# DanielQ-51/cudapathtracer

Hardware: AMD Instinct MI355X
Metric: Mray/s (higher is better)
Workload: dtype f32; 1 GPU; cornell_1920x1080_1024spp_depth8_mis; spp=1024, max_depth=8, integrator=UNIDIRECTIONAL (MIS), variant=megakernel, seed=103033, triangles=36, bvh_nodes=31

## Files before the change

cudapathtracer_amd/api.py:

```python
from __future__ import annotations

import ctypes as C
import os

import numpy as np

_HERE = os.path.dirname(os.path.abspath(__file__))
LIB_PATH = os.environ.get("PT_LIB_PATH") or os.path.join(_HERE, "csrc", "libptamd.so")

UNIDIRECTIONAL = 0
NAIVE_UNIDIRECTIONAL = 2
SEED = 103033
INFO_KEYS = ("width", "height", "spp", "max_depth", "integrator", "leaf_size", "n_tris", "n_lights", "n_nodes",
             "n_points", "n_normals", "n_uvs", "n_mats", "largest_leaf", "backup_count", "tree_depth")
COUNTER_KEYS = ("rays_closest", "rays_shadow", "node_pops", "box_tests", "tri_tests", "hits", "rng_draws", "iterations")


class _F4(C.Union):
    _fields_ = [("v", C.c_float * 4), ("_align", C.c_longdouble)]


class Camera(C.Structure):

    _fields_ = [("cameraOrigin", _F4), ("w", C.c_int32), ("h", C.c_int32), ("xRot", C.c_float), ("yRot", C.c_float),
# ... 140 lines not shown
    L.pt_preview_motion.argtypes = [vp]
    L.pt_preview_set_motion_chain.argtypes = [vp, i32]
    L.pt_preview_motion_chain.argtypes = [vp]
    L.pt_render_ids.argtypes = [vp, C.POINTER(Camera), i32, i32, i32, vp]
    L.pt_render_ids_device.argtypes = [vp, C.POINTER(Camera), i32, i32, i32, vp, vp]
    L.pt_pick.argtypes = [vp, C.POINTER(Camera), i32, i32, i32, vp, i32, vp, vp]
    L.pt_select_overlay.argtypes = [i32, i32, vp, i32, C.POINTER(SelectEntry), vp]
    L.pt_select_overlay_device.argtypes = [i32, i32, vp, i32, C.POINTER(SelectEntry), vp, vp]
    L.pt_preview_set_selection.argtypes = [vp, i32, C.POINTER(SelectEntry), i32]
    L.pt_preview_pick.argtypes = [vp, i32, i32, i32, vp, vp]
    L.pt_preview_read_ids.argtypes = [vp, vp]
    L.pt_preview_device_ids.restype = vp; L.pt_preview_device_ids.argtypes = [vp]
    L.pt_preview_id_passes.argtypes = [vp]
    L.pt_debug_update_ms.argtypes = [vp, vp]
    L.pt_light_triangles.argtypes = [C.POINTER(SceneDesc), vp]
    L.pt_scene_destroy.argtypes = [vp]
    L.pt_render.argtypes = [vp, C.POINTER(Camera), i32, i32, i32, i32, i32, i32, u64, C.POINTER(TileRange), vp]
    L.pt_render_counted.argtypes = [vp, C.POINTER(Camera), i32, i32, i32, i32, i32, i32, u64, C.POINTER(TileRange), vp, vp]
    L.pt_render_tiles_device.argtypes = [vp, C.POINTER(Camera), i32, i32, i32, i32, i32, i32, u64, C.POINTER(TileRange), vp, i32, vp]
    L.pt_untile_device.argtypes = [i32, i32, C.POINTER(TileRange), vp, vp, vp]
    L.pt_tile_device.argtypes = [i32, i32, C.POINTER(TileRange), vp, vp, vp]
    L.pt_launch_unidirectional.argtypes = [i32, Camera, vp, i32, i32, i32, i32, vp]
    L.pt_launch_naive_unidirectional.argtypes = [i32, Camera, vp, i32, i32, i32, i32, vp]
    L.pt_set_variant.argtypes = [vp, i32]
    L.pt_has_experimental.restype = i32
    L.pt_get_counters.argtypes = [vp, vp]
    L.pt_reset_counters.argtypes = [vp]
    L.pt_last_kernel_ms.restype = f32; L.pt_last_kernel_ms.argtypes = [vp]
    L.pt_scene_flags.argtypes = [vp]
    L.pt_last_tile_handovers.argtypes = [vp]
    L.pt_last_moments_launches.argtypes = [vp]
    L.pt_queue_stalls.argtypes = [vp]
    L.pt_debug_queue_header.argtypes = [vp, C.POINTER(C.c_int)]
    L.pt_set_culling.argtypes = [vp, i32]
    L.pt_set_option.argtypes = [vp, C.c_char_p, i32]
    L.pt_get_option.argtypes = [vp, C.c_char_p, vp]
    L.pt_debug_stamps.argtypes = [vp, vp]
    L.pt_rank_tiles.argtypes = [i32, i32, i32, i32, C.POINTER(TileRange)]
    L.pt_multi_create.restype = vp; L.pt_multi_create.argtypes = [C.POINTER(SceneDesc), i32, vp]
    L.pt_multi_destroy.argtypes = [vp]
    L.pt_multi_set_option.argtypes = [vp, C.c_char_p, i32]
    L.pt_multi_set_variant.argtypes = [vp, i32]
    L.pt_multi_render.argtypes = [vp, C.POINTER(Camera), i32, i32, i32, i32, i32, i32, u64, vp, vp]
    L.pt_render_multi.argtypes = [C.POINTER(SceneDesc), i32, vp, C.POINTER(Camera), i32, i32, i32, i32, i32, i32, u64, vp, vp]
    L.pt_probe_rng.argtypes = [u64, i32, vp, i32, vp, vp, vp]
    L.pt_probe_math.argtypes = [i32, vp, vp, vp, vp, vp, vp]
    L.pt_probe_rcp_exhaustive.argtypes = [vp, vp]
    L.pt_probe_camera_rays.argtypes = [C.POINTER(Camera), u64, i32, vp, vp]
    L.pt_probe_trace_closest.argtypes = [vp, i32, vp, vp, vp, vp]
    L.pt_probe_trace_shadow.argtypes = [vp, i32, vp, vp, vp, vp]
    L.pt_probe_bsdf_sample.argtypes = [vp, i32, vp, vp, vp, f32, f32, u64, vp, vp]
    L.pt_probe_bsdf_eval.argtypes = [vp, i32, vp, vp, vp, f32, f32, vp]
    L.novum_scene_load.restype = vp; L.novum_scene_load.argtypes = [C.c_char_p, C.c_char_p, i32]
    L.novum_scene_load_ex.restype = vp; L.novum_scene_load_ex.argtypes = [C.c_char_p, C.c_char_p, i32, i32]
    L.pt_bvh_build_device.argtypes = [vp, i32, vp, i32, i32, i32, vp, i32, vp, vp]
    L.novum_bvh_build_host.argtypes = [vp, i32, vp, i32, i32, vp, i32, vp, vp]
    L.novum_scene_free.argtypes = [vp]
    L.novum_scene_info.argtypes = [vp, vp]
    L.novum_scene_desc.argtypes = [vp, C.POINTER(SceneDesc)]
    L.novum_scene_camera.argtypes = [vp, C.POINTER(Camera)]
    L.novum_make_camera.argtypes = [i32, vp, vp, f32, f32, f32, i32, i32, C.POINTER(Camera)]
    L.novum_finalise.argtypes = [vp, i32, i32]
    L.novum_init_render.argtypes = [C.c_char_p, C.c_char_p, i32, vp, C.c_char_p]
    L.novum_init_render_progressive.argtypes = [C.c_char_p, C.c_char_p, i32, vp, C.c_char_p, C.c_char_p, C.c_char_p, C.c_double, i32]
    L.novum_save_csv_mono.argtypes = [C.c_char_p, vp, i32, i32, i32]
    L.pt_launch_progressive.argtypes = [i32, i32, Camera, vp, i32, i32, i32, i32, vp, i32, PROGRESS_FN, vp]
# ... 555 lines not shown
        out = np.zeros(8, np.uint64)
        _check(lib().pt_debug_stamps(self.h, _p(out)), "pt_debug_stamps")
        return dict(zip(("regen", "closest", "bounce_logic", "wave_lifetimes", "not_earliest_start", "latest_end", "shadow_in_bounce", "slot7"), (int(v) for v in out)))

    def global_node_fetches(self):
        out = np.zeros(8, np.uint64)
        _check(lib().pt_debug_stamps(self.h, _p(out)), "pt_debug_stamps")
        return int(out[0])

    def debug_lane_util(self):
        out = np.zeros(8, np.uint64)
        _check(lib().pt_debug_stamps(self.h, _p(out)), "pt_debug_stamps")
        v = [int(x) for x in out]
        names = ("closest_nodes", "closest_tris", "shadow_nodes", "shadow_tris")
        return {n: {"wave_trips": v[2 * k], "lane_trips": v[2 * k + 1], "lanes_per_trip": (v[2 * k + 1] / v[2 * k]) if v[2 * k] else 0.0}
                for k, n in enumerate(names)}

    def set_culling(self, on=True):
        _check(lib().pt_set_culling(self.h, int(bool(on))), "pt_set_culling")
        return self

    def flags(self):
        f = lib().pt_scene_flags(self.h)
        return {"onchip": bool(f & 1), "persistent": bool(f & 2), "time_slices": bool(f & 4), "hbm_kernel": bool(f & 8), "culling": bool(f & 16), "refill": bool(f & 32), "flat": bool(f & 64), "simple": bool(f & 128), "flat_pair": bool(f & 256), "leaf_table": bool(f & 512), "lean": bool(f & 1024)}

    def tile_handovers(self):
        n = lib().pt_last_tile_handovers(self.h)
        _check(min(n, 0), "pt_last_tile_handovers")
        return n

    def last_moments_launches(self):
        return int(lib().pt_last_moments_launches(self.h))

    def queue_header(self):
        out = (C.c_int * 16)()
        rc = lib().pt_debug_queue_header(self.h, out)
        if rc < 0:
            _check(rc, "pt_debug_queue_header")
        return list(out) if rc == 1 else None

    def queue_stalls(self):
        return int(lib().pt_queue_stalls(self.h))

    def last_kernel_ms(self):
        ms = float(lib().pt_last_kernel_ms(self.h))
        if ms < 0.0:
            raise PtError("pt_last_kernel_ms: " + (lib().pt_last_error().decode(errors="replace") or "the last launch failed"))
        return ms

    def trace_closest(self, rays):
        rays = np.ascontiguousarray(rays, np.float32).reshape(-1, 6)
        n = len(rays)
        oi = np.zeros((n, 4), np.int32); of = np.zeros((n, 12), np.float32); cnt = np.zeros(8, np.uint64)
        _check(lib().pt_probe_trace_closest(self.h, n, _p(rays), _p(oi), _p(of), _p(cnt)), "pt_probe_trace_closest")
        return oi, of, dict(zip(COUNTER_KEYS, (int(v) for v in cnt)))

    def trace_shadow(self, rays, max_t):
        rays = np.ascontiguousarray(rays, np.float32).reshape(-1, 6)
        max_t = np.ascontiguousarray(max_t, np.float32)
        n = len(rays)
        of = np.zeros((n, 3), np.float32); cnt = np.zeros(8, np.uint64)
        _check(lib().pt_probe_trace_shadow(self.h, n, _p(rays), _p(max_t), _p(of), _p(cnt)), "pt_probe_trace_shadow")
        return of, dict(zip(COUNTER_KEYS, (int(v) for v in cnt)))

    def bsdf_sample(self, material, wi, backface, subseq, eta_i=1.0, eta_t=1.0, seed=SEED):
        material = np.ascontiguousarray(material, np.int32); wi = np.ascontiguousarray(wi, np.float32).reshape(-1, 3)
# ... 834 lines not shown
```

cudapathtracer_amd/csrc/pt_api.hip:

```cpp
#include <algorithm>
#include <chrono>
#include <cmath>
#include <cstdarg>
#include <cstdio>
#include <cstdlib>
#include <cstring>
#include <mutex>
#include <string>
#include <vector>

#include "../../include/pt_api.h"
#include "pt_params.h"
#include "pt_feature_host.h"
#include "pt_bvh_build.h"
#include "xorwow_host.h"

using namespace pt;

static_assert(sizeof(pt_bvh_node) == 48 && sizeof(pt_triangle) == 80 && sizeof(pt_material) == 176 && sizeof(pt_camera) == 112,
              "boundary structs must keep the reference's CUDA layouts (SURVEY.md Appendix A)");
static_assert(offsetof(pt_triangle, emission) == 48 && offsetof(pt_triangle, lightInd) == 64, "Triangle layout");
static_assert(offsetof(pt_material, type) == 32 && offsetof(pt_material, albedo) == 48 && offsetof(pt_material, eta) == 80 &&
              offsetof(pt_material, ior) == 112 && offsetof(pt_material, isSpecular) == 128 && offsetof(pt_material, absorption) == 144 &&
              offsetof(pt_material, priority) == 160, "Material layout");
// ... 34 lines not shown
    int nWide = 0, wideStackNeed = 0; bool wideTried = false, wideWanted = false;
    int nLeaves = 0;
    DevBuf rng, spill, tilebuf, colors, pixcnt, queue, left;
    DevBuf wfState, wfCtl, wfCtr, wfSpill;
    DevBuf aovSpill, aovOut;
    DevBuf adS, adM, adH, adList, adKeep, adCount, adOut, adSpp, adErr;
    DevBuf adP, adQ, adSq;
    DevBuf moS, moP, moQ, moOut;
    DevBuf moList;
    int variant = 0;
    int numCU = 256;
    DeviceScene ds{};
    int stackNeed = 0, nInternal = 0, cacheNodes = 0, cacheTris = 0;
    int nMats = 0, nLightsPacked = 0, nTexels = 0;
    bool armless = false;
    int schedMask = 31;
    bool sliceAlways = true;
    bool wavesHbmOk = PT_WAVES_HBM > 0;
    int nodeKeep = 10, triKeep = 8;
    int spec = 2;
    int refill = 1, refillKeep = 6;
    bool refillKeepSet = false;
    bool cull = false;
    unsigned long long lightTri8 = 0ull;
    bool leafBoxes = true;
    int flat2Wanted = 1; int lastLaunchFlat2 = 0;
    bool noLeafTris = false;
    int queueTimeoutMs = 30000;
    int queueStalls = 0;
    bool leanOk = false, leanWanted = true;
    int lastLaunchLean = 0;
    bool momentsFused = false;
    int lastMomentsLaunches = -1;
    bool simpleOk = false, simpleWanted = true;
    bool flatOk = false; int flatWanted = 1;
    int lastLaunchFlat = 0, lastLaunchSimple = 0, lastLaunchLeafTable = 0;
    bool lastLaunchQueued = false;
    int lastLaunchTiles = 0;
    int lastLaunchPushed = 0;
    int lastLaunchRefill = 0;
    int lastLaunchHbm = -1;
    bool wavesHbmForce = false;
    bool onchipOk = true;
    int nTrisPacked = 0;
    int sliceIters = 512;
    int lptPrio = 2;
    bool persistent = true;
    bool xcdBands = false;
    bool deferShadow = false;
    int generation = 0;
    int deviceLeaf = -1;
    int nPositions = 0, nNormals = 0, nUvs = 0;
    DevBuf kTris, kNormals, kUvs, kTypes, kLightTris;
    DevBuf spNodes, spTris, spAttrs, spLights, spLeaves, spNormals;
    DevBuf buildPool;
    DevBuf posCur, posPrev;
    bool hasMotion = false;
    DevBuf motionOut;
    DevBuf idsOut;
    DevBuf edit;
    float renumberMs = 0.0f, updateMs = 0.0f;
    float lastKernelMs = 0.0f;
    bool evPending = false;
    hipEvent_t ev0 = nullptr, ev1 = nullptr;
};

// ... 9 lines not shown
            geom + rec + (size_t)wg * perWave <= (size_t)160 * 1024 * wg / 16) return wg;
    return 0;
}
static bool scene_onchip(const pt_scene* s) { return scene_onchip_wg(s) > 0; }
static bool hbm_kernel_pays(const pt_scene* s, bool simple, long long tiles) {
    if (scene_onchip(s) || (s->deferShadow && !s->armless) || !s->wavesHbmOk) return false;
    const long long slots = (long long)s->numCU * 4 * (simple ? kWavesHbmSimple : kWavesHbm);
    return s->wavesHbmForce || tiles * 4 >= slots * (simple ? 3 : 5);
}

extern "C" {

int pt_fail_(int code, const char* msg) { g_err = msg; return code; }

int pt_api_version(void) { return PT_API_VERSION; }
const char* pt_last_error(void) { return g_err.c_str(); }

int pt_device_count(void) {
    int n = 0;
    hipError_t e = hipGetDeviceCount(&n);
    if (e != hipSuccess) return fail(-2, "hipGetDeviceCount: %s", hipGetErrorString(e));
    return n;
}

void pt_scene_destroy(pt_scene* s) {
    if (!s) return;
    DevBuf* all[] = {&s->nodes, &s->tris, &s->attrs, &s->lights, &s->mats, &s->textures, &s->jump, &s->totals, &s->leaves, &s->wnodes, &s->qnodes, &s->leafBox, &s->mids,
                     &s->rng, &s->spill, &s->tilebuf, &s->colors, &s->pixcnt, &s->queue, &s->left, &s->wfState, &s->wfCtl, &s->wfCtr, &s->wfSpill,
                     &s->aovSpill, &s->aovOut, &s->adS, &s->adM, &s->adH, &s->adList, &s->adKeep, &s->adCount, &s->adOut, &s->adSpp, &s->adErr,
                     &s->adP, &s->adQ, &s->adSq,
                     &s->moS, &s->moP, &s->moQ, &s->moOut, &s->moList,
                     &s->kTris, &s->kNormals, &s->kUvs, &s->kTypes, &s->kLightTris,
                     &s->spNodes, &s->spTris, &s->spAttrs, &s->spLights, &s->spLeaves, &s->spNormals, &s->buildPool,
                     &s->posCur, &s->posPrev, &s->motionOut, &s->idsOut, &s->edit};
    for (DevBuf* b : all) b->release();
    if (s->ev0) (void)hipEventDestroy(s->ev0);
    if (s->ev1) (void)hipEventDestroy(s->ev1);
    delete s;
}

static double wall_ms() { return std::chrono::duration<double, std::milli>(std::chrono::steady_clock::now().time_since_epoch()).count(); }

static int upload(DevBuf& b, const void* src, size_t bytes) {
    if (int r = b.ensure(std::max<size_t>(bytes, 16))) return r;
    if (bytes) HIP_OK(hipMemcpy(b.p, src, bytes, hipMemcpyHostToDevice));
    return 0;
}

static bool boxes_nested_and_finite(const std::vector<PNode>& pn, int nInternal) {
    for (int i = 0; i < nInternal; i++) {
        const PNode& p = pn[i];
        for (int a = 0; a < 3; a++)
            if (!(std::isfinite(p.lmin[a]) && std::isfinite(p.lmax[a]) && std::isfinite(p.rmin[a]) && std::isfinite(p.rmax[a]))) return false;
        const int32_t ref[2] = {p.left, p.right};
        for (int k = 0; k < 2; k++) {
            if (ref[k] < 0) continue;
            if (ref[k] <= i || ref[k] >= nInternal) return false;
            const PNode& c = pn[ref[k]];
            const float* mn = k == 0 ? p.lmin : p.rmin; const float* mx = k == 0 ? p.lmax : p.rmax;
            for (int a = 0; a < 3; a++)
                if (!(mn[a] <= c.lmin[a] && mn[a] <= c.rmin[a] && mx[a] >= c.lmax[a] && mx[a] >= c.rmax[a])) return false;
        }
    }
    return true;
}

extern "C++" {
template <class LightIndOf>
// ... 857 lines not shown
            ok = ok && dec(q.lmin[a]) <= p.lmin[a] && dec(q.lmax[a]) >= p.lmax[a] && dec(q.rmin[a]) <= p.rmin[a] && dec(q.rmax[a]) >= p.rmax[a];
        }
        int mn[2], mx[2];
        uint32_t word[2];
        const int32_t ref[2] = {p.left, p.right};
        for (int c = 0; c < 2 && ok; c++) {
            if (ref[c] >= 0) {
                ok = ref[c] > i && ref[c] < nI;
                if (ok) { mn[c] = minFirst[ref[c]]; mx[c] = maxFirst[ref[c]]; word[c] = (uint32_t)ref[c]; }
            } else {
                const int f = ~ref[c];
                ok = ref[c] != kRefNone && f >= 0 && f < nT;
                if (!ok) break;
                mn[c] = mx[c] = f; word[c] = 0x80000000u | (uint32_t)f;
                const float* bmn = c == 0 ? p.lmin : p.rmin; const float* bmx = c == 0 ? p.lmax : p.rmax;
                float* o = &lb[(size_t)f * 8];
                o[0] = bmn[0]; o[1] = bmn[1]; o[2] = bmn[2]; o[3] = bmx[0]; o[4] = bmx[1]; o[5] = bmx[2];
            }
        }
        if (!ok) break;
        q.left = word[0] | ((uint32_t)(k + 64) << 24); q.right = word[1];
        ok = mx[0] < mn[1];
        minFirst[i] = mn[0]; maxFirst[i] = mx[1]; mids[i] = mn[1];
    }
    if (!ok) return 0;
    if (int r = upload(s->qnodes, qn.data(), qn.size() * sizeof(QNode))) return r;
    if (int r = upload(s->leafBox, lb.data(), lb.size() * sizeof(float))) return r;
    if (int r = upload(s->mids, mids.data(), mids.size() * sizeof(int32_t))) return r;
    s->compactOk = true;
    return 0;
}
#endif

struct FusedMoments { float4* P; float4* Q; int c; bool launched, seeded; };
static int render_tiles(pt_scene* s, const pt_camera* cam, int w, int h, int spp, int maxDepth, int integrator, int useMIS,
                        uint64_t seed, const TileSpan& t, void* d_tiles, uint32_t* d_pixcnt, bool count, hipStream_t stream, bool continueStreams,
                        const int* list = nullptr, int live = -1, FusedMoments* fused = nullptr) {
    if (t.count == 0) return 0;
    if (fused && s->variant == 1) return 0;
    if (!list) live = t.count;
    if (list && (count || s->variant != 0 || t.first != 0 || t.stride != 1 || live < 0 || live > t.count)) return fail(-1, "render_tiles: bad tile list");
    if (int r = s->rng.ensure((size_t)t.count * 384 * sizeof(uint32_t))) return r;
    if (!continueStreams) HIP_OK(launch_rng_init((const uint32_t*)s->jump.p, seed, w, h, t, (uint32_t*)s->rng.p, stream));
    if (fused) fused->seeded = !continueStreams;
    if (s->variant == 1) return render_tiles_wavefront(s, cam, w, h, spp, maxDepth, integrator, useMIS, t, d_tiles, d_pixcnt, count, stream);
    const bool deferred = s->deferShadow && !s->armless;
    const bool onchip = scene_onchip(s) && !deferred;
    const bool simpleTimed = s->simpleOk && s->simpleWanted && s->refill && !s->cull && !s->armless;
    const bool simpleHbm = !onchip && !deferred && s->wavesHbmOk && simpleTimed && !count;
    const bool hbm = hbm_kernel_pays(s, simpleHbm, live);
    KParams P;
    P.onchip = onchip ? 1 : 0;
    P.hbm = hbm ? 1 : 0;
    bool wide = false, compact = false;
#ifdef PT_EXPERIMENTAL
    if (hbm && simpleHbm && s->wideWanted) {
        if (int r = ensure_wide(s)) return r;
        wide = s->nWide > 0;
    }
    if (hbm && simpleHbm && s->compactWanted && !wide) {
        if (int r = ensure_compact(s)) return r;
        compact = s->compactOk;
    }
#endif
    P.wide = wide ? 1 : 0; P.compact = compact ? 1 : 0;
    P.xcdBands = s->xcdBands ? 1 : 0;
    P.cull = (s->cull && hbm) ? 1 : 0;
    P.refill = (s->refill && !deferred && !P.cull && !s->armless && (!onchip || s->refill == 2)) ? 1 : 0;
    P.flat = 0;
    if (onchip && s->flatOk && s->flatWanted && !deferred && !P.refill) {
        P.flat = (s->nInternal <= 64 && s->nTrisPacked <= 64) ? 1 : 2;
    }
    P.simple = ((P.flat && s->simpleOk && s->simpleWanted) || simpleHbm) ? 1 : 0;
    if (P.flat == 1 && s->noLeafTris && !s->armless && s->flat2Wanted && integrator == PT_UNIDIRECTIONAL && !count && useMIS) P.flat = 3;
    P.lean = (s->leanOk && s->leanWanted && !s->armless && !P.simple && !count && !P.cull && (P.flat == 3 || (!onchip && P.refill))) ? 1 : 0;
    const MkRow* row = megakernel_choose(integrator, count, !deferred, P, false);
// ... 748 lines not shown
}

static int queue_error(pt_scene* s) {
    if (!s->queue.p || s->variant != 0 || !s->lastLaunchQueued) return 0;
    int q[8] = {0, 0, 0, 0, 0, 0, 0, 0};
    if (hipMemcpy(q, s->queue.p, sizeof(q), hipMemcpyDeviceToHost) != hipSuccess) return fail(-2, "tile queue read-back failed");
    return queue_words_error(s, q, s->lastLaunchTiles);
}
static int queue_words_error(pt_scene* s, const int* q, int tiles) {
    if (q[3] != 0) {
        if (q[2] >= tiles) { s->queueStalls++; return 0; }
        return fail(-4, "megakernel tile queue timed out (code %d): %d of %d tiles finished, %d pops and %d pushes claimed; the first stalled waiter saw %d finished after %.1f M ticks "
                        "of the device's steady counter without progress: the frame is incomplete", q[3], q[2], tiles, q[0], q[1], q[6], (double)q[7] * 1.048576);
    }
    return 0;
}

int pt_last_tile_handovers(pt_scene* s) {
    if (!s) return fail(-1, "null scene");
    if (!s->queue.p || s->variant != 0 || !s->lastLaunchQueued) return 0;
    int q[4] = {0, 0, 0, 0};
    HIP_OK(hipMemcpy(q, s->queue.p, sizeof(q), hipMemcpyDeviceToHost));
    return std::max(0, q[1] - s->lastLaunchPushed);
}

int pt_debug_queue_header(pt_scene* s, int* out16) {
    if (!s || !out16) return fail(-1, "null argument");
    for (int i = 0; i < kQueueHeader; i++) out16[i] = 0;
    if (!s->queue.p || s->variant != 0 || !s->lastLaunchQueued) return 0;
    HIP_OK(hipMemcpy(out16, s->queue.p, kQueueHeader * sizeof(int), hipMemcpyDeviceToHost));
    return 1;
}

int pt_last_moments_launches(pt_scene* s) { return s ? s->lastMomentsLaunches : -1; }

int pt_queue_stalls(pt_scene* s) { return s ? s->queueStalls : 0; }

int pt_set_culling(pt_scene* s, int on) {
    if (!s) return fail(-1, "null scene");
    s->cull = on != 0;
    return 0;
}

namespace {
struct OptionRef { const char* name; int lo, hi; };
const OptionRef kOptions[] = {
    {"flat", 0, 2}, {"onchip", 0, 1}, {"waves_hbm", 0, 2}, {"refill", 0, 2}, {"refill_keep", 0, 15}, {"node_keep", 0, 15}, {"tri_keep", 0, 15},
    {"defer_shadow", 0, 1}, {"slice_iters", 0, 1 << 30}, {"slice_always", 0, 1}, {"sched_mask", 0, 1 << 20}, {"lpt_prio", 0, 2},
    {"persistent", 0, 1}, {"xcd_bands", 0, 1}, {"culling", 0, 1}, {"spec", 0, 2}, {"simple", 0, 1}, {"flat2", 0, 1}, {"leaf_boxes", 0, 1}, {"wide", 0, 1},
    {"compact", 0, 1}, {"wf_wide_wg", 0, 2}, {"lean", 0, 1}, {"queue_timeout_ms", 0, 1 << 22},
    {"moments_fused", 0, 1},
};
int option_index(const char* name) {
    if (!name) return -1;
    for (size_t i = 0; i < sizeof(kOptions) / sizeof(kOptions[0]); i++) if (!strcmp(kOptions[i].name, name)) return (int)i;
    return -1;
}
}

int pt_set_option(pt_scene* s, const char* name, int v) {
    const int k = option_index(name);
    if (k < 0) return fail(-1, "pt_set_option: unknown option '%s'", name ? name : "(null)");
    if (v < kOptions[k].lo || v > kOptions[k].hi) return fail(-1, "pt_set_option: %s = %d is outside [%d, %d]", name, v, kOptions[k].lo, kOptions[k].hi);
    if (!s) return fail(-1, "pt_set_option: null scene");
#ifndef PT_EXPERIMENTAL
    {
        const bool exp = ((k == 7 || k == 13 || k == 19 || k == 20) && v != 0) || (k == 3 && v == 2) || (k == 15 && v != 2);
        if (exp) return fail(-3, "pt_set_option: %s = %d selects an experimental kernel; rebuild with `make EXPERIMENTAL=1` (pt_has_experimental() == 0)", name, v);
    }
#endif
    switch (k) {
        case 0: s->flatWanted = v; break;
        case 1: s->onchipOk = v != 0; break;
        case 2: s->wavesHbmOk = v != 0 && PT_WAVES_HBM > 0; s->wavesHbmForce = s->wavesHbmOk && v == 2; break;
        case 3: s->refill = v; break;
        case 4: s->refillKeep = v; s->refillKeepSet = true; break;
        case 5: s->nodeKeep = v; break;
        case 6: s->triKeep = v; break;
        case 7: s->deferShadow = v != 0; break;
        case 8: s->sliceIters = v; break;
        case 9: s->sliceAlways = v != 0; break;
        case 10: if (((v + 1) & v) != 0) return fail(-1, "pt_set_option: sched_mask must be 2^k - 1"); s->schedMask = v; break;
        case 11: s->lptPrio = v; break;
        case 12: s->persistent = v != 0; break;
        case 13: s->xcdBands = v != 0; break;
        case 14: s->cull = v != 0; break;
        case 15: s->spec = v; break;
        case 16: s->simpleWanted = v != 0; break;
        case 17: s->flat2Wanted = v; break;
        case 18: s->leafBoxes = v != 0; break;
        case 19: s->wideWanted = v != 0; break;
        case 20: s->compactWanted = v != 0; break;
        case 21: s->wfWideWg = v; break;
        case 22: s->leanWanted = v != 0; break;
        case 23: s->queueTimeoutMs = v; break;
        case 24: s->momentsFused = v != 0; break;
    }
    return 0;
}

int pt_get_option(pt_scene* s, const char* name, int* out) {
    if (option_index(name) < 0) return fail(-1, "pt_get_option: unknown option '%s'", name ? name : "(null)");
    if (!s || !out) return fail(-1, "pt_get_option: null argument");
    switch (option_index(name)) {
        case 0: *out = s->flatWanted; break;
        case 1: *out = s->onchipOk; break;
        case 2: *out = s->wavesHbmForce ? 2 : (s->wavesHbmOk ? 1 : 0); break;
        case 3: *out = s->refill; break;
        case 4: *out = s->refillKeep; break;
        case 5: *out = s->nodeKeep; break;
        case 6: *out = s->triKeep; break;
        case 7: *out = s->deferShadow; break;
        case 8: *out = s->sliceIters; break;
        case 9: *out = s->sliceAlways; break;
        case 10: *out = s->schedMask; break;
        case 11: *out = s->lptPrio; break;
        case 12: *out = s->persistent; break;
        case 13: *out = s->xcdBands; break;
        case 14: *out = s->cull; break;
        case 15: *out = s->spec; break;
        case 16: *out = s->simpleWanted; break;
        case 17: *out = s->flat2Wanted; break;
        case 18: *out = s->leafBoxes; break;
        case 19: *out = s->wideWanted; break;
        case 20: *out = s->compactWanted; break;
        case 21: *out = s->wfWideWg; break;
        case 22: *out = s->leanWanted; break;
        case 23: *out = s->queueTimeoutMs; break;
        case 24: *out = s->momentsFused; break;
        default: return fail(-1, "pt_get_option: unknown option '%s'", name ? name : "(null)");
    }
    return 0;
}

int pt_scene_flags(pt_scene* s) {
    if (!s) return 0;
    const bool onchip = scene_onchip(s);
    const bool pers = s->persistent && !s->xcdBands;
    const bool hbm = s->lastLaunchHbm >= 0 ? s->lastLaunchHbm == 1 : hbm_kernel_pays(s, false, 1ll << 40);
    return (onchip ? 1 : 0) | (pers ? 2 : 0) | ((pers && s->sliceIters > 0) ? 4 : 0) | (hbm ? 8 : 0) | ((s->cull && hbm) ? 16 : 0) | (s->lastLaunchRefill ? 32 : 0) | (s->lastLaunchFlat ? 64 : 0) | (s->lastLaunchSimple ? 128 : 0) | (s->lastLaunchFlat2 ? 256 : 0) | (s->lastLaunchLeafTable ? 512 : 0) | (s->lastLaunchLean ? 1024 : 0);
}

float pt_last_kernel_ms(pt_scene* s) {
    if (!s) return -1.0f;
    if (s->evPending) {
        if (hipEventSynchronize(s->ev1) != hipSuccess || hipEventElapsedTime(&s->lastKernelMs, s->ev0, s->ev1) != hipSuccess) return -1.0f;
        s->evPending = false;
        if (queue_error(s)) return -1.0f;
    }
    return s->lastKernelMs;
}

int pt_host_alloc_zero_(void** p, size_t bytes) {
    HIP_OK(hipMalloc(p, std::max<size_t>(bytes, 16)));
    HIP_OK(hipMemset(*p, 0, bytes));
    return 0;
}
int pt_host_download_(void* d, void* h, size_t bytes) {
    HIP_OK(hipMemcpy(h, d, bytes, hipMemcpyDeviceToHost));
    return 0;
}
int pt_host_download_free_(void* d, void* h, size_t bytes) {
// ... 211 lines not shown
```

cudapathtracer_amd/csrc/pt_kernels.hip:

```cpp
#include "pt_megakernel.h"

namespace pt {



__global__ void __launch_bounds__(256) rng_init_kernel(const uint32_t* __restrict__ jump, unsigned long long seed, int w, int h,
                                                       int tileFirst, int tileStride, int tileCount, int tilesX, uint32_t* __restrict__ rng) {
    int wave = threadIdx.x >> 6, lane = threadIdx.x & 63;
    int lt = blockIdx.x * 4 + wave;
    if (lt >= tileCount) return;
    int tile = tileFirst + lt * tileStride;
    int x = (tile % tilesX) * 8 + (lane & 7), y = (tile / tilesX) * 8 + (lane >> 3);
    uint32_t s0 = (uint32_t)seed ^ 0xaad26b49u, s1 = (uint32_t)(seed >> 32) ^ 0xf7dcefddu;
    uint32_t t0 = 1099087573u * s0, t1 = 2591861531u * s1;
    uint32_t v[5] = {123456789u + t0, 362436069u ^ t0, 521288629u + t1, 88675123u ^ t1, 5783321u + t0};
    uint32_t d = 6615241u + t1 + t0;
    uint32_t idx = (x < w && y < h) ? (uint32_t)(y * w + x) : 0u;
    for (int k = 0; k < 32; k++) {
        if (!__ballot((idx >> k) & 1u)) continue;
        if ((idx >> k) & 1u) {
            const uint32_t* M = jump + (size_t)k * 800;
            uint32_t r[5] = {0, 0, 0, 0, 0};
            for (int i = 0; i < 5; i++) {
                uint32_t word = v[i];
                for (int j = 0; j < 32; j++) {
                    uint32_t m = 0u - ((word >> j) & 1u);
                    const uint32_t* row = M + (i * 32 + j) * 5;
                    r[0] ^= row[0] & m; r[1] ^= row[1] & m; r[2] ^= row[2] & m; r[3] ^= row[3] & m; r[4] ^= row[4] & m;
                }
            }
            for (int i = 0; i < 5; i++) v[i] = r[i];
        }
    }
    uint32_t* o = rng + (size_t)lt * 384 + lane;
    o[0] = v[0]; o[64] = v[1]; o[128] = v[2]; o[192] = v[3]; o[256] = v[4]; o[320] = d;
}

__global__ void queue_init_kernel(int* q, int mask, int nTiles, unsigned long long timeout) {
    int i = blockIdx.x * blockDim.x + threadIdx.x;
    if (i == 0) { q[0] = 0; q[1] = nTiles; q[2] = 0; q[3] = 0; q[4] = 0; q[5] = 0; q[6] = 0; q[7] = 0; ((unsigned long long*)q)[4] = timeout; }
    if (i <= mask)
        ((unsigned long long*)(q + kQueueHeader))[i] = i < nTiles ? (((unsigned long long)(unsigned)(i | kFreshBit) << 32) | (unsigned long long)(i + 1)) : (unsigned long long)i;
}
__global__ void queue_init_list_kernel(int* q, int mask, int nTiles, const int* __restrict__ list, int nList, unsigned long long timeout) {
    int i = blockIdx.x * blockDim.x + threadIdx.x;
    if (i == 0) { q[0] = 0; q[1] = nList; q[2] = nTiles - nList; q[3] = 0; q[4] = 0; q[5] = 0; q[6] = 0; q[7] = 0; ((unsigned long long*)q)[4] = timeout; }
    if (i <= mask)
        ((unsigned long long*)(q + kQueueHeader))[i] = i < nList ? (((unsigned long long)(unsigned)(list[i] | kFreshBit) << 32) | (unsigned long long)(i + 1)) : (unsigned long long)i;
}

__global__ void __launch_bounds__(256) untile_kernel(int w, int h, int tileFirst, int tileStride, int tileCount, int tilesX,
                                                     const float4* __restrict__ tiles, float4* __restrict__ colors) {
    int lt = blockIdx.x * 4 + (threadIdx.x >> 6), lane = threadIdx.x & 63;
    if (lt >= tileCount) return;
    int tile = tileFirst + lt * tileStride;
    int x = (tile % tilesX) * 8 + (lane & 7), y = (tile / tilesX) * 8 + (lane >> 3);
    if (x < w && y < h) colors[(size_t)y * w + x] = tiles[(size_t)lt * 64 + lane];
}
__global__ void __launch_bounds__(256) tile_kernel(int w, int h, int tileFirst, int tileStride, int tileCount, int tilesX,
                                                   const float4* __restrict__ colors, float4* __restrict__ tiles) {
    int lt = blockIdx.x * 4 + (threadIdx.x >> 6), lane = threadIdx.x & 63;
    if (lt >= tileCount) return;
    int tile = tileFirst + lt * tileStride;
    int x = (tile % tilesX) * 8 + (lane & 7), y = (tile / tilesX) * 8 + (lane >> 3);
    tiles[(size_t)lt * 64 + lane] = (x < w && y < h) ? colors[(size_t)y * w + x] : make_float4(0, 0, 0, 0);
}

__global__ void probe_rng_kernel(const uint32_t* __restrict__ jump, unsigned long long seed, int n, const uint32_t* __restrict__ subseq,
                                 int nDraws, uint32_t* outState, uint32_t* outU32, float* outUni) {
    int i = blockIdx.x * blockDim.x + threadIdx.x;
// ... 103 lines not shown

__global__ void probe_bsdf_sample_kernel(DeviceScene S, int n, const int* material, const float* wi3, const int* backface, float etaI,
                                         const uint32_t* __restrict__ state6, float* out8) {
    int i = blockIdx.x * blockDim.x + threadIdx.x;
    if (i >= n) return;
    Rng r = {state6[i * 6], state6[i * 6 + 1], state6[i * 6 + 2], state6[i * 6 + 3], state6[i * 6 + 4], state6[i * 6 + 5]};
    Ctr c = {};
    V3 wo = v3(0.0f), f = v3(0.0f); float pdf = 0.0f;
    sample_f_eval<true>(r, S.mats[material[i]], S.textures, v3(wi3[3 * i], wi3[3 * i + 1], wi3[3 * i + 2]), etaI, backface[i] != 0, wo, f, pdf, 0.0f, 0.0f, c);
    float* o = out8 + 8 * i;
    o[0] = wo.x; o[1] = wo.y; o[2] = wo.z; o[3] = f.x; o[4] = f.y; o[5] = f.z; o[6] = pdf; o[7] = (float)c.draws;
}

__global__ void probe_bsdf_eval_kernel(DeviceScene S, int n, const int* material, const float* wi3, const float* wo3, float etaI, float* out4) {
    int i = blockIdx.x * blockDim.x + threadIdx.x;
    if (i >= n) return;
    const PMat& m = S.mats[material[i]];
    V3 wi = v3(wi3[3 * i], wi3[3 * i + 1], wi3[3 * i + 2]), wo = v3(wo3[3 * i], wo3[3 * i + 1], wo3[3 * i + 2]);
    V3 f = f_eval(m, S.textures, wi, wo, etaI, 0.0f, 0.0f);
    float pdf = 0.0f;
    pdf_eval(m, S.textures, wi, wo, etaI, 0.0f, 0.0f, pdf);
    out4[4 * i] = f.x; out4[4 * i + 1] = f.y; out4[4 * i + 2] = f.z; out4[4 * i + 3] = pdf;
}

}

namespace pt {

hipError_t launch_rng_init(const uint32_t* jump, unsigned long long seed, int w, int h, TileSpan t, uint32_t* rng, hipStream_t stream) {
    if (t.count <= 0) return hipSuccess;
    hipLaunchKernelGGL(rng_init_kernel, dim3((t.count + 3) / 4), dim3(256), 0, stream, jump, seed, w, h, t.first, t.stride, t.count, t.tilesX, rng);
    return hipGetLastError();
}

const MkRow* megakernel_choose(int integrator, bool count, bool syncShadow, const KParams& P, bool moments) {
#ifdef PT_EXPERIMENTAL
    if (moments) return nullptr;
#endif
    if ((integrator != 0 && integrator != 2) || (unsigned)P.flat > 3u) return nullptr;
    int flat = count ? 0 : P.flat;
    if (flat == 3 && integrator != 0) flat = 1;
    const bool simple = P.simple && !count, defer = !syncShadow && integrator != 2;
    const unsigned key = (integrator == 2 ? kMkI2 : 0u) | (count ? kMkCount : 0u) | (defer ? kMkDefer : 0u) | ((P.onchip && !P.hbm) ? kMkLds : 0u) | (P.hbm ? kMkHbm : 0u) |
                         kMkFlat * (unsigned)flat | (simple ? kMkSimple : 0u) | (P.lean ? kMkLean : 0u) | (P.refill ? kMkRefill : 0u) | (P.cull ? kMkCull : 0u) |
                         (P.wide ? kMkWide : 0u) | (P.compact ? kMkCompact : 0u) | (moments ? kMkMoments : 0u);
    for (int i = 0; i < kMkRowsLdsCount; i++) if ((kMkRowsLds[i].key & ~kMkBuiltOnly) == key) return &kMkRowsLds[i];
    for (int i = 0; i < kMkRowsHbmCount; i++) if ((kMkRowsHbm[i].key & ~kMkBuiltOnly) == key) return &kMkRowsHbm[i];
    return nullptr;
}

bool megakernel_has_moments_twin(int integrator, bool count, bool syncShadow, const KParams& P) {
    const MkRow* row = megakernel_choose(integrator, count, syncShadow, P, true);
    return row && !(row->key & kMkBuiltOnly);
}

hipError_t launch_megakernel(const MkRow& row, const KParams& P, int live, const int* list, hipStream_t stream, const MomentsK* M) {
    if (live <= 0) return hipSuccess;
    if ((row.key & kMkBuiltOnly) || ((row.key & kMkMoments) ? !(M && M->c > 0) : M != nullptr)) return hipErrorInvalidValue;
    if (list && !(P.queue && P.gridBlocks > 0)) return hipErrorInvalidValue;
    int nBlocks = megakernel_blocks(live, P.wgWaves);
    if (P.queue && P.gridBlocks > 0) {
        nBlocks = std::min(nBlocks, P.gridBlocks);
        if (list) hipLaunchKernelGGL(queue_init_list_kernel, dim3((P.queueMask + 256) / 256), dim3(256), 0, stream, P.queue, P.queueMask, P.tileCount, list, live, P.queueTimeout);
        else hipLaunchKernelGGL(queue_init_kernel, dim3((P.queueMask + 256) / 256), dim3(256), 0, stream, P.queue, P.queueMask, P.tileCount, P.queueTimeout);
    }
    const unsigned lds = (unsigned)megakernel_lds_bytes(P.cacheNodes, P.cacheTris, row.f.stackEntries, P.wgWaves,
// ... 66 lines not shown
```

cudapathtracer_amd/csrc/pt_params.h:

```cpp
#pragma once
#include "pt_device.h"

namespace pt {

#ifndef PT_STACK_LDS
#define PT_STACK_LDS 16
#endif
#ifndef PT_MIN_WAVES
#define PT_MIN_WAVES 4
#endif
#ifndef PT_CACHE_BYTES
#define PT_CACHE_BYTES 12288
#endif
#ifndef PT_SPEC
#define PT_SPEC 0
#endif
constexpr int kStackLds = PT_STACK_LDS;
#ifndef PT_WAVES_HBM
#define PT_WAVES_HBM 6
#endif
constexpr int kWavesHbm = PT_WAVES_HBM > 0 ? PT_WAVES_HBM : 6;
#ifndef PT_STACK_LDS_HBM
#define PT_STACK_LDS_HBM 8
#endif
// ... 112 lines not shown
    uint32_t* rng;
    float4* out;
    int n, w, h, tileFirst, tileStride, tilesX;
    int nodeKeep, triKeep;
};
size_t wf_state_bytes(int n);
void wf_carve(WfParams& W, void* base);
hipError_t launch_wf_init(const WfParams& W, int spp, hipStream_t s);
hipError_t launch_wf_finish(const WfParams& W, hipStream_t s);
hipError_t launch_wf_logic(int integrator, bool count, bool simple, const WfParams& W, const DeviceScene& S, const CamK& cam, int maxDepth, int useMIS, int it, hipStream_t s);
hipError_t launch_wf_trace(bool count, int wgWaves, int blocks, const WfParams& W, const DeviceScene& S, int cacheNodes, int cacheTris, int32_t* spill, int spillPerLane, int it, hipStream_t s);
hipError_t launch_wf_counters(const WfParams& W, uint32_t* pixCounters, unsigned long long* totals, hipStream_t s);

struct MkFacts {
    int stackEntries;
    bool mediumStacks;
    bool attrCache;
    int wgWaves;
    int wavesPerSimd;
};
enum : unsigned {
    kMkI2 = 1u, kMkCount = 2u, kMkDefer = 4u, kMkLds = 8u, kMkHbm = 16u, kMkFlat = 32u , kMkSimple = 128u, kMkLean = 256u,
    kMkRefill = 512u, kMkCull = 1024u, kMkWide = 2048u, kMkCompact = 4096u, kMkMoments = 8192u,
    kMkBuiltOnly = 16384u
};
struct MkRow { const void* fn; const char* name; MkFacts f; unsigned key; };
#define PT_MK_ROW(KEY, K, ...) MkRow{reinterpret_cast<const void*>(&K<__VA_ARGS__>), #K "<" #__VA_ARGS__ ">", K##_facts<__VA_ARGS__>, (KEY)}
#define PT_MK_ROW2(KEY, K, ...) PT_MK_ROW(KEY, K, 0, ##__VA_ARGS__), PT_MK_ROW((KEY) | kMkI2, K, 2, ##__VA_ARGS__)
extern const MkRow kMkRowsLds[]; extern const int kMkRowsLdsCount;
extern const MkRow kMkRowsHbm[]; extern const int kMkRowsHbmCount;
const MkRow* megakernel_choose(int integrator, bool count, bool syncShadow, const KParams& P, bool moments);

hipError_t launch_rng_init(const uint32_t* jump, unsigned long long seed, int w, int h, TileSpan t, uint32_t* rng, hipStream_t stream);
hipError_t launch_megakernel(const MkRow& row, const KParams& P, int live, const int* list, hipStream_t stream, const MomentsK* M = nullptr);
bool megakernel_has_moments_twin(int integrator, bool count, bool syncShadow, const KParams& P);
hipError_t launch_untile(int w, int h, TileSpan t, const float4* tiles, float4* colors, hipStream_t stream);
hipError_t launch_tile(int w, int h, TileSpan t, const float4* colors, float4* tiles, hipStream_t stream);
hipError_t launch_probe_rng(const uint32_t* jump, unsigned long long seed, int n, const uint32_t* subseq, int nDraws,
                            uint32_t* outState, uint32_t* outU32, float* outUni, hipStream_t stream);
hipError_t launch_probe_math(int n, const float* x, float* s, float* c, float* e, float* rs, float* p5, hipStream_t stream);
hipError_t launch_probe_camera(const uint32_t* state6, const CamK& cam, int n, const int* xy, float* out, hipStream_t stream);
hipError_t launch_probe_rcp_exhaustive(unsigned long long* out3, uint32_t* firstBad, hipStream_t stream);
hipError_t launch_probe_closest(const DeviceScene& S, int n, const float* rays, int32_t* outI, float* outF,
                                unsigned long long* totals, int32_t* spill, hipStream_t stream);
hipError_t launch_probe_shadow(const DeviceScene& S, int n, const float* rays, const float* maxT, float* outF,
                               unsigned long long* totals, int32_t* spill, hipStream_t stream);
hipError_t launch_probe_bsdf_sample(const DeviceScene& S, int n, const int* material, const float* wi3, const int* backface, float etaI,
                                    const uint32_t* state6, float* out8, hipStream_t stream);
hipError_t launch_probe_bsdf_eval(const DeviceScene& S, int n, const int* material, const float* wi3, const float* wo3, float etaI,
                                  float* out4, hipStream_t stream);
inline int probe_trace_blocks(int n) { return (n + 63) / 64; }
inline int megakernel_blocks(int tileCount, int wgWaves = 4) { return (tileCount + wgWaves - 1) / wgWaves; }
inline size_t attr_cache_bytes(int nAttrs, int nMats, int nLights) { return (size_t)nAttrs * 80 + (size_t)nMats * 96 + (size_t)nLights * 64; }
inline size_t megakernel_lds_bytes(int cacheNodes, int cacheTris, int stackEntries = kStackLds, int wgWaves = 4, size_t attrBytes = 0, bool mediumStacks = true) {
    return (size_t)cacheNodes * 64 + (size_t)cacheTris * 48 + (size_t)wgWaves * ((size_t)stackEntries * 256 + (mediumStacks ? (size_t)kMediumMax * 64 : 0)) + attrBytes;
}

}
```

include/pt_api.h:

```cpp
#ifndef PT_API_H
#define PT_API_H

#include <stddef.h>
#include <stdint.h>

#ifdef __cplusplus
extern "C" {
#endif

#define PT_API_VERSION 1
#define PT_TILE_DIM 8
#define PT_TILE_PIXELS 64

typedef struct pt_float4 { float x, y, z, w; } __attribute__((aligned(16))) pt_float4;
typedef struct pt_float2 { float x, y; } __attribute__((aligned(8))) pt_float2;

typedef struct pt_bvh_node {
    pt_float4 aabbMIN, aabbMAX;
    int32_t left, right, first, primCount;
} pt_bvh_node;

typedef struct pt_triangle {
    int32_t aInd, bInd, cInd;
    int32_t naInd, nbInd, ncInd;
// ... 55 lines not shown

pt_scene* pt_scene_create(const pt_scene_desc* desc);
void pt_scene_destroy(pt_scene* scene);

int pt_render(pt_scene* scene, const pt_camera* camera, int w, int h, int spp, int max_depth,
              int integrator, int use_mis, uint64_t seed, const pt_tile_range* tiles, float* out_rgba_sum);

int pt_render_tiles_device(pt_scene* scene, const pt_camera* camera, int w, int h, int spp, int max_depth,
                           int integrator, int use_mis, uint64_t seed, const pt_tile_range* tiles,
                           void* d_tile_rgba, int count_work, void* stream);
int pt_untile_device(int w, int h, const pt_tile_range* tiles, const void* d_tile_rgba, void* d_colors, void* stream);
int pt_tile_device(int w, int h, const pt_tile_range* tiles, const void* d_colors, void* d_tile_rgba, void* stream);

int pt_launch_unidirectional(int maxDepth, pt_camera camera, pt_scene* scene, int numSample, int useMIS, int w, int h, void* d_colors);
int pt_launch_naive_unidirectional(int maxDepth, pt_camera camera, pt_scene* scene, int numSample, int useMIS, int w, int h, void* d_colors);

typedef int (*pt_progress_fn)(int samples_done, void* user);
int pt_launch_progressive(int integrator, int maxDepth, pt_camera camera, pt_scene* scene, int numSample, int useMIS, int w, int h,
                          void* d_colors, int chunk_spp, pt_progress_fn progress, void* user);

int pt_render_counted(pt_scene* scene, const pt_camera* camera, int w, int h, int spp, int max_depth,
                      int integrator, int use_mis, uint64_t seed, const pt_tile_range* tiles,
                      float* out_rgba_sum, uint32_t* out_counters);

int pt_set_variant(pt_scene* scene, int variant);

int pt_get_counters(pt_scene* scene, pt_counters* out);
int pt_reset_counters(pt_scene* scene);
float pt_last_kernel_ms(pt_scene* scene);
int pt_last_tile_handovers(pt_scene* scene);
int pt_queue_stalls(pt_scene* scene);
int pt_last_moments_launches(pt_scene* scene);
int pt_debug_queue_header(pt_scene* scene, int* out16);
int pt_scene_flags(pt_scene* scene);
int pt_set_culling(pt_scene* scene, int on);
int pt_set_option(pt_scene* scene, const char* name, int value);
int pt_get_option(pt_scene* scene, const char* name, int* value);
int pt_has_experimental(void);
int pt_debug_stamps(pt_scene* scene, unsigned long long* out8);

#define PT_MULTI_MAX_DEVICES 16
typedef struct pt_multi pt_multi;
typedef struct pt_multi_stats {
    int32_t n_devices;
    int32_t gather;
    float kernel_ms[PT_MULTI_MAX_DEVICES];
    float render_ms, gather_ms, total_ms;
} pt_multi_stats;
void pt_rank_tiles(int w, int h, int rank, int world, pt_tile_range* out);
pt_multi* pt_multi_create(const pt_scene_desc* desc, int n_devices, const int* device_ids);
void pt_multi_destroy(pt_multi* m);
int pt_multi_set_option(pt_multi* m, const char* name, int value);
int pt_multi_set_variant(pt_multi* m, int variant);
int pt_multi_render(pt_multi* m, const pt_camera* camera, int w, int h, int spp, int max_depth, int integrator, int use_mis,
                    uint64_t seed, float* out_rgba_sum, pt_multi_stats* stats);
int pt_render_multi(const pt_scene_desc* desc, int n_devices, const int* device_ids, const pt_camera* camera, int w, int h, int spp,
                    int max_depth, int integrator, int use_mis, uint64_t seed, float* out_rgba_sum, pt_multi_stats* stats);

int pt_render_aovs(pt_scene* scene, const pt_camera* camera, int w, int h, int aov_spp, uint64_t seed,
                   float* out_albedo, float* out_normal_depth);
int pt_render_aovs_device(pt_scene* scene, const pt_camera* camera, int w, int h, int aov_spp, uint64_t seed,
                          void* d_albedo, void* d_normal_depth, void* stream);

int pt_render_aovs_chain(pt_scene* scene, const pt_camera* camera, int w, int h, int aov_spp, int max_links, uint64_t seed,
                         float* out_albedo, float* out_normal_depth, float* out_links );
int pt_render_aovs_chain_device(pt_scene* scene, const pt_camera* camera, int w, int h, int aov_spp, int max_links, uint64_t seed,
// ... 330 lines not shown
```

Baseline: 31220 Mray/s.

## Seed RNG streams from cached column-jump and row-state tables

```diff
diff --git a/cudapathtracer_amd/api.py b/cudapathtracer_amd/api.py
--- a/cudapathtracer_amd/api.py
+++ b/cudapathtracer_amd/api.py
@@ -196,6 +196,7 @@
     L.pt_last_moments_launches.argtypes = [vp]
     L.pt_queue_stalls.argtypes = [vp]
     L.pt_debug_queue_header.argtypes = [vp, C.POINTER(C.c_int)]
+    L.pt_debug_seed_streams.argtypes = [vp, i32, i32, u64, C.POINTER(TileRange), vp, vp]
     L.pt_set_culling.argtypes = [vp, i32]
     L.pt_set_option.argtypes = [vp, C.c_char_p, i32]
     L.pt_get_option.argtypes = [vp, C.c_char_p, vp]
@@ -817,6 +818,13 @@
     def last_moments_launches(self):
         return int(lib().pt_last_moments_launches(self.h))
 
+    def seed_streams(self, w, h, seed=SEED, tiles=None, stream=0):
+        count = tiles.count if tiles is not None else n_tiles(w, h)
+        out = np.zeros((count, 6, 64), np.uint32)
+        _check(lib().pt_debug_seed_streams(self.h, w, h, seed, C.byref(tiles) if tiles is not None else None, stream or None, _p(out)),
+               "pt_debug_seed_streams")
+        return out
+
     def queue_header(self):
         out = (C.c_int * 16)()
         rc = lib().pt_debug_queue_header(self.h, out)
diff --git a/cudapathtracer_amd/csrc/pt_api.hip b/cudapathtracer_amd/csrc/pt_api.hip
--- a/cudapathtracer_amd/csrc/pt_api.hip
+++ b/cudapathtracer_amd/csrc/pt_api.hip
@@ -90,6 +90,11 @@
     int lastLaunchLean = 0;
     bool momentsFused = false;
     int lastMomentsLaunches = -1;
+    bool rngSeedTables = true;
+    DevBuf colJump, rowState;
+    int colTiles = 0;
+    bool rowValid = false; uint64_t rowSeed = 0; int rowW = 0, rowH = 0;
+    hipEvent_t seedEv = nullptr; hipStream_t seedStream = nullptr;
     bool simpleOk = false, simpleWanted = true;
     bool flatOk = false; int flatWanted = 1;
     int lastLaunchFlat = 0, lastLaunchSimple = 0, lastLaunchLeafTable = 0;
@@ -165,8 +170,9 @@
                      &s->moS, &s->moP, &s->moQ, &s->moOut, &s->moList,
                      &s->kTris, &s->kNormals, &s->kUvs, &s->kTypes, &s->kLightTris,
                      &s->spNodes, &s->spTris, &s->spAttrs, &s->spLights, &s->spLeaves, &s->spNormals, &s->buildPool,
-                     &s->posCur, &s->posPrev, &s->motionOut, &s->idsOut, &s->edit};
+                     &s->posCur, &s->posPrev, &s->motionOut, &s->idsOut, &s->edit, &s->colJump, &s->rowState};
     for (DevBuf* b : all) b->release();
+    if (s->seedEv) (void)hipEventDestroy(s->seedEv);
     if (s->ev0) (void)hipEventDestroy(s->ev0);
     if (s->ev1) (void)hipEventDestroy(s->ev1);
     delete s;
@@ -1090,6 +1096,32 @@
 }
 #endif
 
+static int seed_streams(pt_scene* s, uint64_t seed, int w, int h, const TileSpan& t, hipStream_t stream) {
+    const uint32_t* jump = (const uint32_t*)s->jump.p;
+    if (!s->rngSeedTables) { HIP_OK(launch_rng_init(jump, seed, w, h, t, (uint32_t*)s->rng.p, stream)); return 0; }
+    if (s->seedEv && stream != s->seedStream) HIP_OK(hipStreamWaitEvent(stream, s->seedEv, 0));
+    bool built = false;
+    if (t.tilesX > s->colTiles) {
+        s->colTiles = 0;
+        if (int r = s->colJump.ensure((size_t)t.tilesX * 800 * sizeof(uint32_t))) return r;
+        HIP_OK(launch_rng_col_jump(jump, t.tilesX, (uint32_t*)s->colJump.p, stream));
+        s->colTiles = t.tilesX; built = true;
+    }
+    if (!s->rowValid || s->rowSeed != seed || s->rowW != w || s->rowH != h) {
+        s->rowValid = false;
+        if (int r = s->rowState.ensure((size_t)h * 40 * sizeof(uint32_t))) return r;
+        HIP_OK(launch_rng_row_state(jump, seed, w, h, (uint32_t*)s->rowState.p, stream));
+        s->rowValid = true; s->rowSeed = seed; s->rowW = w; s->rowH = h; built = true;
+    }
+    if (built) {
+        if (!s->seedEv) HIP_OK(hipEventCreateWithFlags(&s->seedEv, hipEventDisableTiming));
+        HIP_OK(hipEventRecord(s->seedEv, stream));
+        s->seedStream = stream;
+    }
+    HIP_OK(launch_rng_seed((const uint32_t*)s->colJump.p, (const uint32_t*)s->rowState.p, seed, w, h, t, (uint32_t*)s->rng.p, stream));
+    return 0;
+}
+
 struct FusedMoments { float4* P; float4* Q; int c; bool launched, seeded; };
 static int render_tiles(pt_scene* s, const pt_camera* cam, int w, int h, int spp, int maxDepth, int integrator, int useMIS,
                         uint64_t seed, const TileSpan& t, void* d_tiles, uint32_t* d_pixcnt, bool count, hipStream_t stream, bool continueStreams,
@@ -1099,7 +1131,7 @@
     if (!list) live = t.count;
     if (list && (count || s->variant != 0 || t.first != 0 || t.stride != 1 || live < 0 || live > t.count)) return fail(-1, "render_tiles: bad tile list");
     if (int r = s->rng.ensure((size_t)t.count * 384 * sizeof(uint32_t))) return r;
-    if (!continueStreams) HIP_OK(launch_rng_init((const uint32_t*)s->jump.p, seed, w, h, t, (uint32_t*)s->rng.p, stream));
+    if (!continueStreams) { if (int r = seed_streams(s, seed, w, h, t, stream)) return r; }
     if (fused) fused->seeded = !continueStreams;
     if (s->variant == 1) return render_tiles_wavefront(s, cam, w, h, spp, maxDepth, integrator, useMIS, t, d_tiles, d_pixcnt, count, stream);
     const bool deferred = s->deferShadow && !s->armless;
@@ -1914,6 +1946,18 @@
     return 1;
 }
 
+int pt_debug_seed_streams(pt_scene* s, int w, int h, uint64_t seed, const pt_tile_range* tiles, void* stream, uint32_t* out) {
+    if (!s || !out) return fail(-1, "pt_debug_seed_streams: null argument");
+    TileSpan t;
+    if (int r = resolve_tiles(w, h, tiles, t)) return r;
+    if (t.count == 0) return 0;
+    if (int r = s->rng.ensure((size_t)t.count * 384 * sizeof(uint32_t))) return r;
+    if (int r = seed_streams(s, seed, w, h, t, (hipStream_t)stream)) return r;
+    HIP_OK(hipMemcpyAsync(out, s->rng.p, (size_t)t.count * 384 * sizeof(uint32_t), hipMemcpyDeviceToHost, (hipStream_t)stream));
+    HIP_OK(hipStreamSynchronize((hipStream_t)stream));
+    return 0;
+}
+
 int pt_last_moments_launches(pt_scene* s) { return s ? s->lastMomentsLaunches : -1; }
 
 int pt_queue_stalls(pt_scene* s) { return s ? s->queueStalls : 0; }
@@ -1930,7 +1974,7 @@
     {"flat", 0, 2}, {"onchip", 0, 1}, {"waves_hbm", 0, 2}, {"refill", 0, 2}, {"refill_keep", 0, 15}, {"node_keep", 0, 15}, {"tri_keep", 0, 15},
     {"defer_shadow", 0, 1}, {"slice_iters", 0, 1 << 30}, {"slice_always", 0, 1}, {"sched_mask", 0, 1 << 20}, {"lpt_prio", 0, 2},
     {"persistent", 0, 1}, {"xcd_bands", 0, 1}, {"culling", 0, 1}, {"spec", 0, 2}, {"simple", 0, 1}, {"flat2", 0, 1}, {"leaf_boxes", 0, 1}, {"wide", 0, 1},
-    {"compact", 0, 1}, {"wf_wide_wg", 0, 2}, {"lean", 0, 1}, {"queue_timeout_ms", 0, 1 << 22},
+    {"compact", 0, 1}, {"wf_wide_wg", 0, 2}, {"lean", 0, 1}, {"rng_seed", 0, 1}, {"queue_timeout_ms", 0, 1 << 22},
     {"moments_fused", 0, 1},
 };
 int option_index(const char* name) {
@@ -1975,8 +2019,9 @@
         case 20: s->compactWanted = v != 0; break;
         case 21: s->wfWideWg = v; break;
         case 22: s->leanWanted = v != 0; break;
-        case 23: s->queueTimeoutMs = v; break;
-        case 24: s->momentsFused = v != 0; break;
+        case 23: s->rngSeedTables = v != 0; break;
+        case 24: s->queueTimeoutMs = v; break;
+        case 25: s->momentsFused = v != 0; break;
     }
     return 0;
 }
@@ -2008,8 +2053,9 @@
         case 20: *out = s->compactWanted; break;
         case 21: *out = s->wfWideWg; break;
         case 22: *out = s->leanWanted; break;
-        case 23: *out = s->queueTimeoutMs; break;
-        case 24: *out = s->momentsFused; break;
+        case 23: *out = s->rngSeedTables; break;
+        case 24: *out = s->queueTimeoutMs; break;
+        case 25: *out = s->momentsFused; break;
         default: return fail(-1, "pt_get_option: unknown option '%s'", name ? name : "(null)");
     }
     return 0;
diff --git a/cudapathtracer_amd/csrc/pt_kernels.hip b/cudapathtracer_amd/csrc/pt_kernels.hip
--- a/cudapathtracer_amd/csrc/pt_kernels.hip
+++ b/cudapathtracer_amd/csrc/pt_kernels.hip
@@ -36,6 +36,79 @@
     o[0] = v[0]; o[64] = v[1]; o[128] = v[2]; o[192] = v[3]; o[256] = v[4]; o[320] = d;
 }
 
+__device__ __forceinline__ void xorwow_seed_state(unsigned long long seed, uint32_t (&v)[5], uint32_t& d) {
+    uint32_t s0 = (uint32_t)seed ^ 0xaad26b49u, s1 = (uint32_t)(seed >> 32) ^ 0xf7dcefddu;
+    uint32_t t0 = 1099087573u * s0, t1 = 2591861531u * s1;
+    v[0] = 123456789u + t0; v[1] = 362436069u ^ t0; v[2] = 521288629u + t1; v[3] = 88675123u ^ t1; v[4] = 5783321u + t0;
+    d = 6615241u + t1 + t0;
+}
+__device__ __forceinline__ void jump_apply(const uint32_t* __restrict__ M, uint32_t (&v)[5]) {
+    uint32_t r[5] = {0, 0, 0, 0, 0};
+#pragma unroll
+    for (int i = 0; i < 5; i++) {
+#pragma unroll 1
+        for (int half = 0; half < 2; half++) {
+            const uint32_t word = v[i] >> (16 * half);
+            const uint32_t* rows = M + (i * 32 + 16 * half) * 5;
+#pragma unroll
+            for (int j = 0; j < 16; j++) {
+                uint32_t m = 0u - ((word >> j) & 1u);
+                const uint32_t* row = rows + j * 5;
+                r[0] ^= row[0] & m; r[1] ^= row[1] & m; r[2] ^= row[2] & m; r[3] ^= row[3] & m; r[4] ^= row[4] & m;
+            }
+        }
+    }
+    for (int i = 0; i < 5; i++) v[i] = r[i];
+}
+__device__ __forceinline__ void jump_walk(const uint32_t* __restrict__ jump, uint32_t idx, uint32_t (&v)[5]) {
+    for (int k = 0; k < 32; k++) {
+        if (!__ballot((idx >> k) & 1u)) continue;
+        if ((idx >> k) & 1u) jump_apply(jump + (size_t)k * 800, v);
+    }
+}
+
+__global__ void __launch_bounds__(192) rng_col_jump_kernel(const uint32_t* __restrict__ jump, int tilesX, uint32_t* __restrict__ colJump) {
+    const int tx = blockIdx.x, r = threadIdx.x;
+    if (tx >= tilesX) return;
+    uint32_t v[5];
+    for (int q = 0; q < 5; q++) v[q] = (r >> 5) == q ? 1u << (r & 31) : 0u;
+    jump_walk(jump, 8u * (uint32_t)tx, v);
+    if (r >= 160) return;
+    uint32_t* o = colJump + ((size_t)tx * 160 + r) * 5;
+    for (int q = 0; q < 5; q++) o[q] = v[q];
+}
+
+__global__ void __launch_bounds__(64) rng_row_state_kernel(const uint32_t* __restrict__ jump, unsigned long long seed, int w, int h,
+                                                           uint32_t* __restrict__ rowState) {
+    const int i = blockIdx.x * 64 + threadIdx.x, y = i >> 3;
+    uint32_t v[5], d;
+    xorwow_seed_state(seed, v, d);
+    jump_walk(jump, y < h ? (uint32_t)(y * w + (i & 7)) : 0u, v);
+    if (y >= h) return;
+    uint32_t* o = rowState + (size_t)i * 5;
+    for (int q = 0; q < 5; q++) o[q] = v[q];
+}
+
+__global__ void __launch_bounds__(256) rng_seed_kernel(const uint32_t* __restrict__ colJump, const uint32_t* __restrict__ rowState,
+                                                       unsigned long long seed, int w, int h, int tileFirst, int tileStride, int tileCount,
+                                                       int tilesX, uint32_t* __restrict__ rng) {
+    int wave = threadIdx.x >> 6, lane = threadIdx.x & 63;
+    int lt = blockIdx.x * 4 + wave;
+    if (lt >= tileCount) return;
+    int tile = __builtin_amdgcn_readfirstlane(tileFirst + lt * tileStride);
+    int tx = tile % tilesX;
+    int x = tx * 8 + (lane & 7), y = (tile / tilesX) * 8 + (lane >> 3);
+    uint32_t v[5], d;
+    xorwow_seed_state(seed, v, d);
+    if (x < w && y < h) {
+        const uint32_t* s = rowState + ((size_t)y * 8 + (lane & 7)) * 5;
+        for (int q = 0; q < 5; q++) v[q] = s[q];
+        jump_apply(colJump + (size_t)tx * 800, v);
+    }
+    uint32_t* o = rng + (size_t)lt * 384 + lane;
+    o[0] = v[0]; o[64] = v[1]; o[128] = v[2]; o[192] = v[3]; o[256] = v[4]; o[320] = d;
+}
+
 __global__ void queue_init_kernel(int* q, int mask, int nTiles, unsigned long long timeout) {
     int i = blockIdx.x * blockDim.x + threadIdx.x;
     if (i == 0) { q[0] = 0; q[1] = nTiles; q[2] = 0; q[3] = 0; q[4] = 0; q[5] = 0; q[6] = 0; q[7] = 0; ((unsigned long long*)q)[4] = timeout; }
@@ -205,6 +278,22 @@
     hipLaunchKernelGGL(rng_init_kernel, dim3((t.count + 3) / 4), dim3(256), 0, stream, jump, seed, w, h, t.first, t.stride, t.count, t.tilesX, rng);
     return hipGetLastError();
 }
+hipError_t launch_rng_col_jump(const uint32_t* jump, int tilesX, uint32_t* colJump, hipStream_t stream) {
+    if (tilesX <= 0) return hipSuccess;
+    hipLaunchKernelGGL(rng_col_jump_kernel, dim3(tilesX), dim3(192), 0, stream, jump, tilesX, colJump);
+    return hipGetLastError();
+}
+hipError_t launch_rng_row_state(const uint32_t* jump, unsigned long long seed, int w, int h, uint32_t* rowState, hipStream_t stream) {
+    if (h <= 0) return hipSuccess;
+    hipLaunchKernelGGL(rng_row_state_kernel, dim3((h * 8 + 63) / 64), dim3(64), 0, stream, jump, seed, w, h, rowState);
+    return hipGetLastError();
+}
+hipError_t launch_rng_seed(const uint32_t* colJump, const uint32_t* rowState, unsigned long long seed, int w, int h, TileSpan t, uint32_t* rng,
+                           hipStream_t stream) {
+    if (t.count <= 0) return hipSuccess;
+    hipLaunchKernelGGL(rng_seed_kernel, dim3((t.count + 3) / 4), dim3(256), 0, stream, colJump, rowState, seed, w, h, t.first, t.stride, t.count, t.tilesX, rng);
+    return hipGetLastError();
+}
 
 const MkRow* megakernel_choose(int integrator, bool count, bool syncShadow, const KParams& P, bool moments) {
 #ifdef PT_EXPERIMENTAL
diff --git a/cudapathtracer_amd/csrc/pt_params.h b/cudapathtracer_amd/csrc/pt_params.h
--- a/cudapathtracer_amd/csrc/pt_params.h
+++ b/cudapathtracer_amd/csrc/pt_params.h
@@ -168,6 +168,10 @@
 const MkRow* megakernel_choose(int integrator, bool count, bool syncShadow, const KParams& P, bool moments);
 
 hipError_t launch_rng_init(const uint32_t* jump, unsigned long long seed, int w, int h, TileSpan t, uint32_t* rng, hipStream_t stream);
+hipError_t launch_rng_col_jump(const uint32_t* jump, int tilesX, uint32_t* colJump, hipStream_t stream);
+hipError_t launch_rng_row_state(const uint32_t* jump, unsigned long long seed, int w, int h, uint32_t* rowState, hipStream_t stream);
+hipError_t launch_rng_seed(const uint32_t* colJump, const uint32_t* rowState, unsigned long long seed, int w, int h, TileSpan t, uint32_t* rng,
+                           hipStream_t stream);
 hipError_t launch_megakernel(const MkRow& row, const KParams& P, int live, const int* list, hipStream_t stream, const MomentsK* M = nullptr);
 bool megakernel_has_moments_twin(int integrator, bool count, bool syncShadow, const KParams& P);
 hipError_t launch_untile(int w, int h, TileSpan t, const float4* tiles, float4* colors, hipStream_t stream);
diff --git a/include/pt_api.h b/include/pt_api.h
--- a/include/pt_api.h
+++ b/include/pt_api.h
@@ -111,6 +111,7 @@
 int pt_queue_stalls(pt_scene* scene);
 int pt_last_moments_launches(pt_scene* scene);
 int pt_debug_queue_header(pt_scene* scene, int* out16);
+int pt_debug_seed_streams(pt_scene* scene, int w, int h, uint64_t seed, const pt_tile_range* tiles, void* stream, uint32_t* out);
 int pt_scene_flags(pt_scene* scene);
 int pt_set_culling(pt_scene* scene, int on);
 int pt_set_option(pt_scene* scene, const char* name, int value);
```

Result: no change. 31430 Mray/s, median of 6 (+0.7%).
